# aswanthabam/JPEG_Decoder

Hardware: AMD Instinct MI355X
Metric: Mpixels/s decoded (IDCT+colour) (higher is better)
Workload: dtype f32; 1 GPU; stream of 4096x4096 baseline 4:4:4 images, 32 images per step (one launch) per GPU, coefficient blocks resident in HBM; sampling=4:4:4, parallelism=images sharded x1, no collective, launched_by=bench.py

## Files before the change

jpeg_decoder_amd/csrc/jb_api.cpp:

```cpp
#include <atomic>
#include <condition_variable>
#include <deque>
#include <map>
#include <memory>
#include <mutex>
#include <thread>
#include <hip/hip_runtime_api.h>

#include <cstdarg>
#include <chrono>
#include <cstdio>
#include <cstdlib>
#include <cstring>
#include <new>
#include <string>
#include <vector>

#include <sched.h>

#include "../../include/jpegblk.h"
#include "jb_kernels.h"
#include "jb_huff.h"
#include "jb_knobs.h"

// ... 715 lines not shown
    size_t cap = lay.device_total + lay.device_total / 4 + 65536;
    if (cap < ctx->blob_hint) cap = ctx->blob_hint;
    JB_HIP(ctx, hipMalloc(&s.d_blob, cap));
    s.blob_cap = cap;
    ctx->blob_hint = cap;
  }
  if (!s.h_status) {
    JB_HIP(ctx, hipHostMalloc((void **)&s.h_status, 4 * 256, hipHostMallocDefault));
    JB_HIP(ctx, hipMalloc((void **)&s.d_status, 4 * 256));
  }
  if (lay.total <= ((size_t)4 << 20)) JB_HIP(ctx, jbk_huff_fetch(s.d_blob, h, lay.total, up));
  else JB_HIP(ctx, hipMemcpyAsync(s.d_blob, h, lay.total, hipMemcpyHostToDevice, up));
  JB_HIP(ctx, jbk_huff_zero(d_out, zero_bytes, up, s.d_status, 4 * (size_t)lay.n));
  JbHuffLaunch p;
  memset(&p, 0, sizeof p);
  const uint8_t *d = (const uint8_t *)s.d_blob;
  uint8_t *dw = (uint8_t *)s.d_blob;
  p.scan = d + lay.off_scan;
  p.starts = (const uint32_t *)(d + lay.off_starts);
  p.tables = (const JbHuffTables *)(d + lay.off_tab);
  p.images = (const JbHuffImage *)(d + lay.off_img);
  p.wgs = (const JbHuffWg *)(d + lay.off_wg);
  p.sync_wgs = (const JbHuffWg *)(d + lay.off_sync_wg);
  p.coef = d_out;
  p.status = s.d_status;
  p.n_wgs = (int32_t)lay.n_wg;
  p.n_sync_wgs = (int32_t)lay.n_sync_wg;
  p.chunks = (const JbChunkDesc *)(d + lay.off_chunks);
  p.entry = (JbChunkState *)(dw + lay.off_entry);
  p.exit = (JbChunkState *)(dw + lay.off_exit);
  p.cps = (uint32_t *)(dw + lay.off_cps);
  p.chunk_dc = (JbChunkDc *)(dw + lay.off_chunk_dc);
  p.wgsum = (JbWgSum *)(dw + lay.off_wgsum);
  p.n_chunks_total = lay.n_chunks;
  p.sync_launches = lay.n_sync_wg > 0 && lay.n_wg == lay.n ? 1 : sync_launches;
  p.max_chunk_bytes = lay.max_chunk_bytes;
  p.max_tabs = lay.max_tabs;
  JB_HIP(ctx, jbk_huff_launch(p, up));
  return JB_OK;
}

int pack_into_slot(jb_ctx *ctx, Slot &s, const JbHuffJob *const *jobs, int n, int64_t coef_stride, JbHuffLayout *lay) {
  const size_t need = jb_huff_pack_size_(jobs, n);
  if (need > s.h_blob_cap) {
    if (s.h_blob) (void)hipHostFree(s.h_blob);
    s.h_blob = nullptr, s.h_blob_cap = 0;
    const size_t cap = need + need / 4 + 65536;
    JB_HIP(ctx, hipHostMalloc((void **)&s.h_blob, cap, hipHostMallocDefault));
    s.h_blob_cap = cap;
  }
  const int rc = jb_huff_pack_(jobs, n, coef_stride, s.h_blob, lay);
  return rc ? fail(ctx, rc, "submission too large for the device entropy decoder") : JB_OK;
}

int submit_jobs_impl(jb_ctx *ctx, const JbHuffJob *const *jobs, const uint8_t *packed, const JbHuffLayout *lay_in,
                     const jb_image_desc *desc_in, const uint16_t *qtabs_in, int n_images, uint8_t *rgb, int64_t rgb_stride,
                     uint32_t *status_out, int *ticket, bool dst_device = false, int scale = 1, const jb_output_spec *fmt = nullptr) {
  if (ctx->n_slots == 0) return fail(ctx, JB_ERR_CAPACITY, "context was created without staging buffers");
  if (n_images < 1 || n_images > kMaxBatch) return fail(ctx, JB_ERR_GEOMETRY, "n_images = %d outside 1..%d", n_images, kMaxBatch);
  const jb_image_desc *desc = jobs ? &jobs[0]->desc : desc_in;
  jb_geometry g;
  int rc = check_desc(ctx, desc, &g);
  if (rc) return rc;
  int32_t out_w = 0, out_h = 0;
  if (jb_scaled_size(desc->width, desc->height, scale, &out_w, &out_h) != JB_OK) return fail(ctx, JB_ERR_GEOMETRY, "scale %d is not 1, 2, 4 or 8", scale);
  const int64_t out_bytes = 3LL * out_w * out_h * fmt_esize(fmt);
// ... 392 lines not shown
      Entry fresh;
      CPU_ZERO(&fresh.set);
      fresh.n = numa_cpus_for_(device, numa_knob, &fresh.set);
      it = cache.emplace(std::make_pair(device, numa_knob), fresh).first;
    }
    e = it->second;
  }
  if (e.n <= 0) return 0;
  if (sched_setaffinity(0, sizeof e.set, &e.set) != 0) return 0;
  return e.n;
}

void jb_ctx_set_last_desc_(jb_ctx *ctx, const jb_image_desc *d) { ctx->last_desc = *d; }
const JbKnobs *jb_ctx_knobs_(const jb_ctx *ctx) { return &ctx->knobs; }

int jb_fail_(jb_ctx *ctx, int code, const char *msg) { return fail(ctx, code, "%s", msg); }

size_t jb_huff_pack_size_(const JbHuffJob *const *jobs, int n) {
  size_t n_wg = 0, n_starts = 0, scan_bytes = 0, n_chunks = 0;
  for (int i = 0; i < n; i++) {
    n_wg += (jobs[i]->img.n_chunks + kJbOwnChunks - 1) / kJbOwnChunks;
    n_chunks += jobs[i]->img.n_chunks;
    n_starts += jobs[i]->starts.size();
    scan_bytes += ((jobs[i]->scan.size() + 15) & ~(size_t)15);
  }
  return (size_t)n * sizeof(JbHuffImage) + 2 * n_wg * sizeof(JbHuffWg) + (size_t)n * sizeof(JbHuffTables) + n_starts * 4 +
         n_chunks * sizeof(JbChunkDesc) + scan_bytes + 512;
}

int jb_huff_pack_(const JbHuffJob *const *jobs, int n, int64_t coef_stride, uint8_t *h, JbHuffLayout *lay) {
  auto a16 = [](size_t v) { return (v + 15) & ~(size_t)15; };
  std::vector<int> set_of((size_t)n, 0);
  std::vector<int> sets;
  size_t n_wg = 0, n_sync_wg = 0, n_starts = 0, scan_bytes = 0, n_chunks = 0;
  lay->max_chunk_bytes = 0;
  lay->max_tabs = 0;
  for (int i = 0; i < n; i++) {
    int found = -1;
    for (size_t k = 0; k < sets.size() && found < 0; k++)
      if (jobs[sets[k]]->n_tabs == jobs[i]->n_tabs && memcmp(&jobs[sets[k]]->tables, &jobs[i]->tables, sizeof(JbHuffTables)) == 0) found = (int)k;
    if (found < 0) {
      found = (int)sets.size();
      sets.push_back(i);
    }
    set_of[(size_t)i] = found;
    const size_t wgs = (jobs[i]->img.n_chunks + kJbOwnChunks - 1) / kJbOwnChunks;
    n_wg += wgs;
    if (jobs[i]->img.needs_sync) n_sync_wg += wgs;
    n_chunks += jobs[i]->img.n_chunks;
    n_starts += jobs[i]->starts.size();
    scan_bytes += a16(jobs[i]->scan.size());
    if (jobs[i]->img.chunk_bytes > lay->max_chunk_bytes) lay->max_chunk_bytes = jobs[i]->img.chunk_bytes;
    if (jobs[i]->n_tabs > lay->max_tabs) lay->max_tabs = jobs[i]->n_tabs;
    if ((int64_t)jobs[i]->geo.coef_bytes > coef_stride) return JB_ERR_CAPACITY;
  }
  lay->off_img = 0;
  lay->off_wg = a16((size_t)n * sizeof(JbHuffImage));
  lay->off_sync_wg = a16(lay->off_wg + n_wg * sizeof(JbHuffWg));
  lay->off_tab = a16(lay->off_sync_wg + n_sync_wg * sizeof(JbHuffWg));
  lay->off_starts = lay->off_tab + sets.size() * sizeof(JbHuffTables);
  lay->off_chunks = a16(lay->off_starts + n_starts * 4);
  lay->off_scan = a16(lay->off_chunks + n_chunks * sizeof(JbChunkDesc));
  lay->total = lay->off_scan + scan_bytes + 256;
  lay->off_entry = a16(lay->total);
  lay->off_exit = a16(lay->off_entry + n_chunks * sizeof(JbChunkState));
  lay->off_cps = a16(lay->off_exit + n_chunks * sizeof(JbChunkState));
  lay->off_chunk_dc = (a16(lay->off_cps + n_chunks * kJbCheckpoints * 4) + 31) & ~(size_t)31;
  lay->off_wgsum = lay->off_chunk_dc + n_chunks * sizeof(JbChunkDc);
  lay->device_total = a16(lay->off_wgsum + n_wg * sizeof(JbWgSum));
  lay->n = n;
  lay->n_wg = (int)n_wg;
  lay->n_sync_wg = (int)n_sync_wg;
  lay->n_chunks = (uint32_t)n_chunks;
  lay->coef_stride = coef_stride;
  if (lay->device_total > 0xffffff00u || n_wg > 0x7fffffffu || n_chunks > 0x3fffffffu) return JB_ERR_CAPACITY;
  JbHuffImage *im = (JbHuffImage *)(h + lay->off_img);
  JbHuffWg *wg = (JbHuffWg *)(h + lay->off_wg);
  JbHuffWg *swg = (JbHuffWg *)(h + lay->off_sync_wg);
  uint32_t *st = (uint32_t *)(h + lay->off_starts);
  size_t w = 0, sw = 0, si = 0, sc = lay->off_scan, chunk0 = 0;
  for (size_t k = 0; k < sets.size(); k++) memcpy(h + lay->off_tab + k * sizeof(JbHuffTables), &jobs[sets[k]]->tables, sizeof(JbHuffTables));
  for (int i = 0; i < n; i++) {
    const JbHuffJob &j = *jobs[i];
    im[i] = j.img;
    im[i].scan_off = (uint32_t)(sc - lay->off_scan);
    im[i].int_off = (uint32_t)si;
    im[i].table_set = (uint32_t)set_of[(size_t)i];
    im[i].coef_off = (int64_t)i * coef_stride;
    im[i].state_off = (uint32_t)chunk0;
    im[i].wg0 = (uint32_t)w;
    JbChunkDesc *cd = (JbChunkDesc *)(h + lay->off_chunks) + chunk0;
    uint32_t c = 0;
    for (uint32_t seg = 0; seg + 1 < (uint32_t)j.starts.size(); seg++) {
      const uint32_t k = jb_chunks_of_(j.starts[seg + 1] - j.starts[seg], j.img.chunk_bytes);
      if (c + k > j.img.n_chunks) return JB_ERR_STATE;
      for (uint32_t q = 0; q < k; q++) cd[c++] = JbChunkDesc{j.starts[seg] + q * j.img.chunk_bytes, seg | (q == 0 ? 0x80000000u : 0u)};
    }
    if (c != j.img.n_chunks) return JB_ERR_STATE;
    chunk0 += j.img.n_chunks;
    for (uint32_t f = 0; f < j.img.n_chunks; f += kJbOwnChunks) {
      wg[w++] = JbHuffWg{(uint32_t)i, f};
      if (j.img.needs_sync) swg[sw++] = JbHuffWg{(uint32_t)i, f};
    }
    memcpy(st + si, j.starts.data(), j.starts.size() * 4);
    si += j.starts.size();
    memcpy(h + sc, j.scan.data(), j.scan.size());
    sc += a16(j.scan.size());
  }
  memset(h + sc, 0, 256);
  return JB_OK;
}
```

jpeg_decoder_amd/csrc/jb_frontend.cpp:

```cpp
#include <chrono>
#include <cstdio>
#include <cstdlib>
#include <cstring>
#include <memory>
#include <string>
#include <thread>
#include <vector>

#include "../../include/jpegblk.h"
#include "jb_entropy.h"
#include "jb_hostmem.h"
#include "jb_huff.h"
#include "jb_huff_core.h"
#include "jb_knobs.h"

struct jb_ctx;
int jb_fail_(jb_ctx *ctx, int code, const char *msg);
void jb_ctx_set_last_desc_(jb_ctx *ctx, const jb_image_desc *d);
const JbKnobs *jb_ctx_knobs_(const jb_ctx *ctx);
extern "C" int jb_decode_job_(jb_ctx *ctx, const JbHuffJob *job, uint8_t *rgb, int64_t rgb_stride);
extern "C" int jb_decode_job_scaled_(jb_ctx *ctx, const JbHuffJob *job, uint8_t *rgb, int64_t rgb_stride, int scale);
extern "C" int jb_blocks_to_rgb_scaled_(jb_ctx *ctx, const jb_image_desc *desc, const int16_t *coef, const uint16_t *qtabs,
                                        uint8_t *rgb, int64_t rgb_stride, int scale);
extern "C" int jb_decode_job_fmt_(jb_ctx *ctx, const JbHuffJob *job, uint8_t *rgb, int64_t rgb_stride, int scale, const jb_output_spec *fmt);
// ... 279 lines not shown
      const HuffTable &t = is_ac ? fr->ac[ac_ids[q]] : fr->dc[dc_ids[q - n_ac]];
      if (!jb_huff_fill_table_(t.counts, t.symbols, is_ac, &job->tables, (uint32_t)q, job->n_tabs, &n_t2))
        return done(JB_ERR_UNSUPPORTED, "Huffman tables with more long codes than the device decoder's tables hold: host decoder");
    }
  }
  const uint32_t ny = (uint32_t)(fr->desc.hs * fr->desc.vs);
  job->img.nb = fr->ncomp == 1 ? 1u : ny + 2;
  job->img.lut_ac = job->img.lut_dc = job->img.lut_comp = 0;
  for (uint32_t b = 0; b < job->img.nb; b++) {
    const uint32_t c = b < ny ? 0u : b - ny + 1u;
    job->img.lut_ac |= (uint32_t)ac_slot[c] << (4 * b);
    job->img.lut_dc |= (uint32_t)(n_ac + dc_slot[c]) << (4 * b);
    job->img.lut_comp |= c << (4 * b);
  }
  static thread_local CleanScan tls_scan;
  CleanScan &cs = tls_scan;
  unstuff(fr->scan, fr->scan + fr->scan_len, cs);
  if ((int64_t)cs.n_intervals() != n_int) return done(JB_ERR_UNSUPPORTED, "restart markers do not match the frame: host decoder");
  if (cs.start.back() > 0x0ffff000u) return done(JB_ERR_UNSUPPORTED, "scan too large for 32-bit bit offsets: host decoder");
  job->scan_len = cs.start.back();
  job->scan.assign(cs.bytes.begin(), cs.bytes.begin() + (long)(job->scan_len + 64));
  job->starts.resize(cs.start.size());
  for (size_t i = 0; i < cs.start.size(); i++) job->starts[i] = (uint32_t)cs.start[i];
  job->img.scan_off = job->img.int_off = job->img.table_set = 0;
  job->img.scan_len = (uint32_t)job->scan_len;
  job->img.n_int = (uint32_t)n_int;
  job->img.ri = (uint32_t)(ri > 0 ? ri : n_mcus);
  job->img.n_mcus = (uint32_t)n_mcus;
  job->img.coef_off = 0;
  job->img.blk_bytes = fr->ncomp == 1 ? 384u : 128u;
  job->img.wg0 = 0;
  if ((uint64_t)n_mcus * job->img.nb >= (1u << 24)) return done(JB_ERR_UNSUPPORTED, "more blocks than the device decoder's 24-bit block index holds: host decoder");
  job->img.n_blocks = (uint32_t)(n_mcus * job->img.nb);
  const uint32_t chunk_bytes = (chunk_knob == 64 || chunk_knob == 128) ? chunk_knob : kJbChunkBytes;
  job->img.chunk_bytes = chunk_bytes;
  {
    uint64_t n_chunks = 0;
    bool needs_sync = false;
    for (size_t i = 0; i + 1 < job->starts.size(); i++) {
      if (job->starts[i + 1] < job->starts[i]) return done(JB_ERR_FORMAT, "restart intervals out of order");
      const uint32_t k = jb_chunks_of_(job->starts[i + 1] - job->starts[i], chunk_bytes);
      needs_sync |= k > 1;
      n_chunks += k;
    }
    if (n_chunks > 0x3fffffffu) return done(JB_ERR_UNSUPPORTED, "scan too large for the device decoder: host decoder");
    job->img.n_chunks = (uint32_t)n_chunks;
    job->img.needs_sync = needs_sync ? 1u : 0u;
  }
  job->img.state_off = 0;
  if (ri == 0 && job->scan_len == 0) return done(JB_ERR_FORMAT, "empty scan");
  return done(JB_OK, "");
}

extern "C" {

int jb_entropy_decode(const uint8_t *jpeg, size_t jpeg_bytes, jb_image_desc *desc, uint16_t *qtabs,
                      int16_t *coef, size_t coef_cap_bytes) {
  return jb_entropy_decode_mt(jpeg, jpeg_bytes, desc, qtabs, coef, coef_cap_bytes, 1);
}

int jb_entropy_decode_mt(const uint8_t *jpeg, size_t jpeg_bytes, jb_image_desc *desc, uint16_t *qtabs,
                         int16_t *coef, size_t coef_cap_bytes, int n_threads) {
  if (!jpeg || !desc) return jb_fail_(nullptr, JB_ERR_NULL, "jb_entropy_decode: NULL pointer");
  Frame *fr = new Frame();
  Err e;
  int rc = parse_headers(jpeg, jpeg_bytes, *fr, e);
// ... 161 lines not shown
```

jpeg_decoder_amd/csrc/jb_huff.h:

```cpp
#pragma once
#include <stdint.h>

constexpr int kJbT1Bits = 10;
constexpr int kJbT2Bits = 16 - kJbT1Bits;
constexpr uint32_t kJbT1Entries = 1u << kJbT1Bits;
constexpr uint32_t kJbT2Entries = 1u << kJbT2Bits;
constexpr uint32_t kJbT2Tables = 24;
constexpr uint32_t kJbMaxTabs = 6;
struct JbHuffTables {
  uint16_t t1[kJbMaxTabs][kJbT1Entries];
  uint16_t t2[kJbT2Tables][kJbT2Entries];
};
constexpr uint32_t kJbAdvEob = 82;

struct JbHuffImage {
  uint32_t scan_off;
  uint32_t scan_len;
  uint32_t int_off;
  uint32_t n_int;
  uint32_t ri;
  uint32_t n_mcus;
  uint32_t nb;
  uint32_t table_set;
  int64_t coef_off;
  uint32_t lut_ac;
  uint32_t lut_dc;
  uint32_t lut_comp;
  uint32_t n_chunks;
  uint32_t state_off;
  uint32_t n_blocks;
  uint32_t chunk_bytes;
  uint32_t wg0;
  uint32_t needs_sync;
  uint32_t blk_bytes;
  uint32_t n_tabs;
};

struct JbHuffWg {
  uint32_t image;
  uint32_t first_chunk;
};

constexpr uint32_t kJbChunkBytes = 128;
constexpr int kJbHuffLanes = 256;
constexpr uint32_t kJbWarmChunks = 8;
constexpr uint32_t kJbOwnChunks = kJbHuffLanes - kJbWarmChunks;
constexpr int kJbSyncLaunches = 2;
constexpr int kJbSyncLaunchesMax = 8;

inline uint32_t jb_chunks_of_(uint32_t interval_bytes, uint32_t chunk_bytes) { return interval_bytes ? (interval_bytes + chunk_bytes - 1) / chunk_bytes : 1u; }
struct JbChunkDesc {
  uint32_t start;
  uint32_t seg;
};

struct JbChunkState {
  uint32_t bitpos;
  uint32_t meta;
};

constexpr uint32_t kJbCheckpointBits = 256;
constexpr uint32_t kJbCheckpoints = 4;

struct JbWgSum {
  uint32_t has_first;
  uint32_t blocks;
  uint32_t dc[3];
  uint32_t pad[3];
};
struct JbChunkDc {
  uint32_t dc[3];
  uint32_t first_block;
  uint32_t count;
  uint32_t pad[3];
};

struct JbHuffLaunch {
  const uint8_t *scan;
  const uint32_t *starts;
  const JbHuffTables *tables;
  const JbHuffImage *images;
  const JbHuffWg *wgs;
  const JbHuffWg *sync_wgs;
  int16_t *coef;
  uint32_t *status;
  int32_t n_wgs;
  int32_t n_sync_wgs;
  const JbChunkDesc *chunks;
  JbChunkState *entry;
  JbChunkState *exit;
  uint32_t *cps;
  JbChunkDc *chunk_dc;
  JbWgSum *wgsum;
  uint32_t n_chunks_total;
  int32_t sync_launches;
  uint32_t max_chunk_bytes;
  uint32_t max_tabs;
};


#include <string>
#include <vector>

#include "../../include/jpegblk.h"

struct JbHuffJob {
  jb_image_desc desc;
  jb_geometry geo;
  uint16_t qtabs[256];
  JbHuffImage img;
  JbHuffTables tables;
  uint32_t n_tabs = 0;
  std::vector<uint8_t> scan;
  size_t scan_len = 0;
  std::vector<uint32_t> starts;
};
int jb_huff_prepare_(const uint8_t *jpeg, size_t jpeg_bytes, JbHuffJob *job, std::string *err, uint32_t chunk_bytes = 0);

struct JbHuffLayout {
  size_t off_img = 0, off_wg = 0, off_sync_wg = 0, off_tab = 0, off_starts = 0, off_chunks = 0, off_scan = 0, total = 0;
  size_t off_entry = 0, off_exit = 0, off_cps = 0, off_chunk_dc = 0, off_wgsum = 0, device_total = 0;
  int n = 0, n_wg = 0, n_sync_wg = 0;
  uint32_t n_chunks = 0, max_chunk_bytes = 0, max_tabs = 0;
  int64_t coef_stride = 0;
};
inline bool jb_huff_worth_it_(const JbHuffJob &job, uint32_t min_chunks) { return job.img.n_chunks >= min_chunks; }
size_t jb_huff_pack_size_(const JbHuffJob *const *jobs, int n);
int jb_huff_pack_(const JbHuffJob *const *jobs, int n, int64_t coef_stride, uint8_t *dst, JbHuffLayout *lay);
bool jb_huff_fill_table_(const uint8_t counts[17], const uint8_t *symbols, bool is_ac, JbHuffTables *set, uint32_t tix, uint32_t n_tabs, uint32_t *n_t2);
```

jpeg_decoder_amd/csrc/jb_huff.hip:

```cpp
#include <hip/hip_runtime.h>
#include <stdint.h>

#include "jb_huff_core.h"
#include "jb_kernels.h"

namespace {

constexpr uint32_t L = kJbhLanes;
constexpr int kMaxPasses = (int)L + 4;

__constant__ uint8_t kZz2Dev[64] = {0,   2,   16,  32,  18,  4,   6,   20,  34,  48, 64,  50,  36,  22,  8,   10,
                                    24,  38,  52,  66,  80,  96,  82,  68,  54,  40, 26,  12,  14,  28,  42,  56,
                                    70,  84,  98,  112, 114, 100, 86,  72,  58,  44, 30,  46,  60,  74,  88,  102,
                                    116, 118, 104, 90,  76,  62,  78,  92,  106, 120, 122, 108, 94,  110, 124, 126};

template <uint32_t kMaxChunk>
struct Lay {
  static constexpr uint32_t kRows = jbh_rows(kMaxChunk);
  static constexpr uint32_t kNcp = kMaxChunk * 8u / kJbCheckpointBits;
  static_assert(kNcp <= kJbCheckpoints, "records per chunk");
  static constexpr uint32_t off_stream = 0;
  static constexpr uint32_t off_cp = off_stream + kRows * L * 4u;
  static constexpr uint32_t off_xbit = off_cp + kNcp * L * 4u;
  static constexpr uint32_t off_xmeta = off_xbit + L * 4u;
// ... 148 lines not shown
  const bool owned = tid >= kJbWarmChunks && ci < img.n_chunks;
  const bool active = ci < img.n_chunks && (owned || launch == 0);
  const uint32_t gidx = img.state_off + (ci < img.n_chunks ? ci : img.n_chunks - 1u);
  const ChunkGeo g = chunk_geo(p, img, gidx);
  const uint32_t u0 = jbh_u_of_bit(g.start, g.start * 8u), u_end = u0 + (g.end - g.start) * 8u;
  const size_t n_all = p.n_chunks_total;

  JbChunkState entry{g.start * 8u, 0u}, exitst{0u, 0u};
  bool changed = active;
  if (launch > 0) {
    bool c0 = false;
    JbChunkState ne{0u, 0u};
    if (tid == kJbWarmChunks && owned && !g.first) {
      ne = p.exit[gidx - 1u];
      const JbChunkState en = p.entry[gidx];
      c0 = ne.bitpos != en.bitpos || ((ne.meta ^ en.meta) & 0xffffu) != 0;
    }
    if (!__syncthreads_or(c0)) return;
    entry = p.entry[gidx];
    exitst = p.exit[gidx];
    changed = c0;
    if (c0) entry = JbChunkState{ne.bitpos, ne.meta & 0xffffu};
  }
  load_tables(tab, p, img, tid);
  if (active) load_stream<Ly::kRows>(stream, p.scan + img.scan_off, g.start, tid);
#pragma unroll
  for (uint32_t i = 0; i < Ly::kNcp; i++) cpst[i * L + tid] = launch > 0 ? p.cps[i * n_all + gidx] : 0xffffffffu;
  __syncthreads();

  JbhCtx cx;
  cx.scol = stream + tid;
  cx.tab = tab;
  cx.zz2 = nullptr;
  cx.lut_ac = img.lut_ac, cx.lut_dc = img.lut_dc, cx.lut_comp = img.lut_comp;
  cx.nb4 = img.nb * 4u;
  cx.blk_bytes = img.blk_bytes;
  cx.t2_first = img.n_tabs * kJbT1Entries;
  uint32_t *const cpl = cpst + tid;

  for (int pass = 0; pass < kMaxPasses; pass++) {
    if (__builtin_amdgcn_ballot_w64(changed) != 0) {
      JbhLane st;
      {
        const uint32_t bit = entry.bitpos < g.start * 8u ? g.start * 8u : entry.bitpos;
        const uint32_t u = jbh_u_of_bit(g.start, bit);
        st.u = (changed && u < u_end) ? u : u_end;
        st.k = entry.meta & 0xffu;
        st.blk4 = ((entry.meta >> 8) & 0xffu) * 4u;
        if (st.k > 63u) st.k = 0;
        if (st.blk4 >= cx.nb4) st.blk4 = 0;
        st.nblk = 0;
      }
      uint32_t none = 0;
      while (st.u < u_end) {
        const uint32_t up = st.u;
        (void)jbh_step<false>(cx, st, none, none, none, nullptr, 0u);
        if (((st.u ^ up) >> 8) != 0) {
          uint32_t *rec = cpl + ((st.u >> 8) - 1u) * L;
          const uint32_t s = jbh_pack_state(st), old = *rec;
          const bool met = (st.u < u_end) & (((old ^ s) & 0xfffffu) == 0);
          *rec = met ? old : s;
          st.u = met ? (kMet | ((st.u >> 8) - 1u)) : st.u;
        }
      }
      JBH_TRACE_PASS_END(pass);
      if (changed) {
        if (st.u >= kMet) {
// ... 58 lines not shown
  const uint32_t bpi = img.ri * img.nb;

  load_tables(tab, p, img, tid);
  if (tid < 16) ((uint32_t *)misc)[tid] = ((const uint32_t *)kZz2Dev)[tid];
  if (active) load_stream<Ly::kRows>(stream, p.scan + img.scan_off, g.start, tid);

  uint32_t err = 0;
  JbChunkState entry{g.start * 8u, 0u}, want{0u, 0u};
  uint32_t block = g.seg * bpi;
  if (img.needs_sync) {
    Seg mine{0, 0, 0, 0, 0};
    if (active) {
      want = p.exit[gidx];
      mine.f = g.first ? 1u : 0u;
      mine.n = (want.meta >> 16) + (g.first ? g.seg * bpi : 0u);
      if (!g.first) {
        const JbChunkState prev = p.exit[gidx - 1u];
        const JbChunkState en = p.entry[gidx];
        entry = JbChunkState{prev.bitpos, prev.meta & 0xffffu};
        if (en.bitpos != prev.bitpos || ((en.meta ^ prev.meta) & 0xffffu) != 0) err |= 4u;
      }
    }
    const Seg carry = fold_left_workgroups(p, img.wg0, img.wg0 + wg.first_chunk / kJbOwnChunks, misc + 40, tid);
    Seg total;
    const Seg left = scan_left(mine, carry, misc + 16, tid, &total);
    if (!g.first) block = left.n;
  }
  __syncthreads();

  JbhCtx cx;
  cx.scol = stream + tid;
  cx.tab = tab;
  cx.zz2 = (const uint8_t *)misc;
  cx.lut_ac = img.lut_ac, cx.lut_dc = img.lut_dc, cx.lut_comp = img.lut_comp;
  cx.nb4 = img.nb * 4u;
  cx.blk_bytes = img.blk_bytes;
  cx.t2_first = img.n_tabs * kJbT1Entries;

  uint32_t block_end = (g.seg + 1u) * img.ri < img.n_mcus ? (g.seg + 1u) * bpi : img.n_mcus * img.nb;
  if (block_end > img.n_blocks) block_end = img.n_blocks;
  JbhLane st;
  const bool overran = active && entry.bitpos > g.end * 8u;
  {
    const uint32_t bit = entry.bitpos < g.start * 8u ? g.start * 8u : entry.bitpos;
    const uint32_t u = jbh_u_of_bit(g.start, bit);
    st.u = u < u_end ? u : u_end;
    st.k = entry.meta & 0xffu;
    st.blk4 = ((entry.meta >> 8) & 0xffu) * 4u;
    if (st.k > 63u) st.k = 0;
    if (st.blk4 >= cx.nb4) st.blk4 = 0;
    st.nblk = 0;
  }
  const uint32_t k_in = st.k;
  uint32_t dc0 = 0, dc1 = 0, dc2 = 0;
  uint8_t *const coef = (uint8_t *)p.coef + img.coef_off;
  bool live = active && st.u < u_end && block < block_end;
  while (live) {
    if (jbh_step<true>(cx, st, dc0, dc1, dc2, coef, block)) {
      err |= 1u;
      live = false;
    } else {
      live = st.u < u_end && block + st.nblk < block_end;
    }
  }
  JBH_TRACE_PASS_END(0);
  if (active) {
    if (g.last) {
      if (block + st.nblk != block_end || st.k != 0 || st.u > u_end || overran) err |= 2u;
    } else if (img.needs_sync) {
      if (jbh_bit_of_u(g.start, st.u) != want.bitpos || (st.k | (st.blk4 << 6) | ((st.nblk & 0xffffu) << 16)) != want.meta) err |= 4u;
    }
    if (err) atomicOr(p.status + wg.image, err);
    JbChunkDc o;
    o.dc[0] = dc0, o.dc[1] = dc1, o.dc[2] = dc2;
    o.first_block = block + (k_in != 0 ? 1u : 0u);
    o.count = err ? 0u : st.nblk + (st.k != 0 ? 1u : 0u) - (k_in != 0 ? 1u : 0u);
    o.pad[0] = o.pad[1] = o.pad[2] = 0;
    p.chunk_dc[gidx] = o;
  }
  if (img.needs_sync) {
    Seg mine{0, 0, 0, 0, 0};
    if (active) mine = Seg{g.first ? 1u : 0u, 0u, dc0, dc1, dc2};
    Seg total;
    (void)seg_scan_wg(mine, misc + 16, tid, &total);
    if (tid == 0) {
      JbWgSum *o = p.wgsum + img.wg0 + wg.first_chunk / kJbOwnChunks;
      o->dc[0] = total.d0, o->dc[1] = total.d1, o->dc[2] = total.d2;
    }
  }
}

__global__ __launch_bounds__(kJbHuffLanes) void jb_huff_dc_kernel(const JbHuffLaunch p) {
  extern __shared__ __attribute__((aligned(16))) uint8_t lds[];
  uint32_t *const misc = (uint32_t *)lds;
  const uint32_t tid = threadIdx.x;
  const JbHuffWg wg = p.wgs[blockIdx.x];
  const JbHuffImage img = p.images[wg.image];
  const uint32_t ci = wg.first_chunk + tid;
  const bool active = tid < kJbOwnChunks && ci < img.n_chunks;
  const uint32_t gidx = img.state_off + (active ? ci : img.n_chunks - 1u);
  const bool first = (p.chunks[gidx].seg >> 31) != 0;
  JbChunkDc cd = p.chunk_dc[gidx];
  if (!active) cd.count = 0;
  uint32_t p0 = 0, p1 = 0, p2 = 0;
  if (img.needs_sync) {
    Seg mine{0, 0, 0, 0, 0};
    if (active) mine = Seg{first ? 1u : 0u, 0u, cd.dc[0], cd.dc[1], cd.dc[2]};
    const Seg carry = fold_left_workgroups(p, img.wg0, img.wg0 + wg.first_chunk / kJbOwnChunks, misc + 40, tid);
    Seg total;
    const Seg left = scan_left(mine, carry, misc + 16, tid, &total);
    if (!first) p0 = left.d0, p1 = left.d1, p2 = left.d2;
  }
  uint8_t *const coef = (uint8_t *)p.coef + img.coef_off;
  uint32_t pos4 = (cd.first_block % img.nb) * 4u;
  uint32_t bad = 0;
  constexpr uint32_t kBatch = 24;
  for (uint32_t i = 0; i < cd.count; i += kBatch) {
    int32_t diff[kBatch];
#pragma unroll
    for (uint32_t q = 0; q < kBatch; q++) diff[q] = i + q < cd.count ? *(const int16_t *)(coef + (size_t)jbh_mul24(cd.first_block + i + q, img.blk_bytes)) : 0;
#pragma unroll
    for (uint32_t q = 0; q < kBatch; q++) {
      if (i + q < cd.count) {
        const uint32_t c = jbh_ubfe(img.lut_comp, pos4, 4);
        const uint32_t pr = (c == 0 ? p0 : c == 1 ? p1 : p2) + (uint32_t)diff[q];
        bad |= (pr + 32768u) > 65535u ? 1u : 0u;
        p0 = c == 0 ? pr : p0;
        p1 = c == 1 ? pr : p1;
        p2 = c == 2 ? pr : p2;
        *(int16_t *)(coef + (size_t)jbh_mul24(cd.first_block + i + q, img.blk_bytes)) = (int16_t)pr;
        pos4 = pos4 + 4u == img.nb * 4u ? 0u : pos4 + 4u;
      }
    }
  }
  if (bad) atomicOr(p.status + wg.image, 1u);
}

__global__ __launch_bounds__(256) void jb_huff_fetch_kernel(uint4 *dst, const uint4 *src, uint32_t n16) {
  for (uint32_t i = blockIdx.x * 256u + threadIdx.x; i < n16; i += gridDim.x * 256u) dst[i] = src[i];
}
__global__ __launch_bounds__(256) void jb_huff_zero_kernel(uint4 *dst, uint64_t n16, uint4 *small, uint32_t small16) {
  const uint4 z = make_uint4(0, 0, 0, 0);
  if (blockIdx.x == 0 && threadIdx.x < small16) small[threadIdx.x] = z;
  for (uint64_t i = (uint64_t)blockIdx.x * 256u + threadIdx.x; i < n16; i += (uint64_t)gridDim.x * 256u) dst[i] = z;
}
hipError_t jbk_huff_zero(void *d_dst, size_t bytes, hipStream_t stream, void *d_small, size_t small_bytes) {
  (void)hipGetLastError();
  const uint64_t n16 = (bytes + 15) / 16;
  uint64_t blocks = (n16 + 255u) / 256u;
  if (blocks > 8192u) blocks = 8192u;
  const uint32_t small16 = d_small ? (uint32_t)((small_bytes + 15) / 16) : 0u;
  if (small16 > 256u) return hipErrorInvalidValue;
  hipLaunchKernelGGL(jb_huff_zero_kernel, dim3((unsigned)(blocks ? blocks : 1u)), dim3(256), 0, stream, (uint4 *)d_dst, n16, (uint4 *)d_small, small16);
  return hipGetLastError();
}
hipError_t jbk_huff_fetch(void *d_dst, const void *h_pinned_src, size_t bytes, hipStream_t stream) {
  (void)hipGetLastError();
  const uint32_t n16 = (uint32_t)((bytes + 15) / 16);
  unsigned blocks = (n16 + 255u) / 256u;
  if (blocks > 1024u) blocks = 1024u;
  hipLaunchKernelGGL(jb_huff_fetch_kernel, dim3(blocks ? blocks : 1u), dim3(256), 0, stream, (uint4 *)d_dst, (const uint4 *)h_pinned_src, n16);
  return hipGetLastError();
}

// ... 21 lines not shown
```

jpeg_decoder_amd/csrc/jb_huff_core.h:

```cpp
#pragma once
#include <stdint.h>

#include "jb_huff.h"

#if defined(__HIPCC__)
#define JBH_FN __host__ __device__ inline __attribute__((always_inline))
#else
#define JBH_FN inline
#endif

JBH_FN uint32_t jbh_alignbit(uint32_t hi, uint32_t lo, uint32_t sh) {
#if defined(__HIP_DEVICE_COMPILE__)
  return __builtin_amdgcn_alignbit(hi, lo, sh);
#else
  return (uint32_t)(((((uint64_t)hi) << 32) | lo) >> (sh & 31u));
#endif
}
JBH_FN uint32_t jbh_ubfe(uint32_t v, uint32_t off, uint32_t width) {
#if defined(__HIP_DEVICE_COMPILE__)
  return __builtin_amdgcn_ubfe(v, off, width);
#else
  off &= 31u, width &= 31u;
  return width ? (v >> off) & ((1u << width) - 1u) : 0u;
#endif
}
JBH_FN int32_t jbh_sbfe(uint32_t v, uint32_t off, uint32_t width) {
#if defined(__HIP_DEVICE_COMPILE__)
  return __builtin_amdgcn_sbfe((int32_t)v, off, width);
#else
  off &= 31u, width &= 31u;
  if (!width) return 0;
  const uint32_t f = (v >> off) & ((1u << width) - 1u);
  return (int32_t)(f << (32u - width)) >> (32u - width);
#endif
}

JBH_FN uint32_t jbh_mul24(uint32_t a, uint32_t b) { return (a & 0xffffffu) * (b & 0xffffffu); }

#ifndef JBH_TRACE_STEP
#define JBH_TRACE_STEP() ((void)0)
#define JBH_TRACE_PASS_END(pass) ((void)0)
#endif

constexpr uint32_t kJbhLanes = (uint32_t)kJbHuffLanes;
constexpr uint32_t jbh_rows(uint32_t chunk_bytes) { return chunk_bytes / 4u + 3u; }

JBH_FN uint32_t jbh_base_byte(uint32_t start) { return (start & ~3u) - 4u; }
JBH_FN uint32_t jbh_u_of_bit(uint32_t start, uint32_t bit) { return bit - 8u * jbh_base_byte(start) - 1u; }
JBH_FN uint32_t jbh_bit_of_u(uint32_t start, uint32_t u) { return u + 8u * jbh_base_byte(start) + 1u; }

struct JbhCtx {
  const uint32_t *scol;
  const uint16_t *tab;
  const uint8_t *zz2;
  uint32_t lut_ac, lut_dc, lut_comp;
  uint32_t nb4;
  uint32_t blk_bytes;
  uint32_t t2_first;
};
struct JbhLane {
  uint32_t u;
  uint32_t k;
  uint32_t blk4;
  uint32_t nblk;
};

template <bool kStore>
JBH_FN bool jbh_step(const JbhCtx &cx, JbhLane &st, uint32_t &dc0, uint32_t &dc1, uint32_t &dc2, uint8_t *coef, uint32_t block0) {
  JBH_TRACE_STEP();
  const uint32_t u = st.u;
  const uint32_t j = jbh_ubfe(u, 5, 27);
  const uint32_t w = jbh_alignbit(cx.scol[j * kJbhLanes], cx.scol[j * kJbhLanes + kJbhLanes], ~u);
  const bool isdc = st.k == 0;
  const uint32_t tix = jbh_ubfe(isdc ? cx.lut_dc : cx.lut_ac, st.blk4, 4);
  uint32_t e = cx.tab[(tix << kJbT1Bits) + (w >> (32 - kJbT1Bits))];
  if (e - 1u < 31u)
    e = cx.tab[cx.t2_first + ((e - 1u) << kJbT2Bits) + ((w >> 16) & (kJbT2Entries - 1u))];
  const uint32_t total = e & 31u, size = (e >> 5) & 15u, adv = e >> 9;
  const uint32_t k1 = st.k + adv;
  const bool bad = e == 0 || (k1 - 65u) < 17u;
  if (kStore) {
    const int32_t x = jbh_sbfe(w, 32u - total, size);
    const int32_t val = x - (int32_t)(((1u << size) - 1u) ^ (uint32_t)(x >> 31));
    const uint32_t c = jbh_ubfe(cx.lut_comp, st.blk4, 4);
    const uint32_t dcv = (isdc && !bad) ? (uint32_t)val : 0u;
    dc0 += c == 0 ? dcv : 0u;
    dc1 += c == 1 ? dcv : 0u;
    dc2 += c == 2 ? dcv : 0u;
    if (!bad && (isdc || size != 0))
      *(int16_t *)(coef + (jbh_mul24(block0 + st.nblk, cx.blk_bytes) + cx.zz2[k1 - 1u])) = (int16_t)val;
  }
  const uint32_t k2 = k1 - ((size == 0 && !isdc) ? 1u : 0u);
  const bool done = k2 >= 64u;
  const bool next = done || bad;
  st.k = next ? 0u : k2;
  st.nblk += (done && !bad) ? 1u : 0u;
  const uint32_t b4 = st.blk4 + (next ? 4u : 0u);
  st.blk4 = b4 == cx.nb4 ? 0u : b4;
  st.u = u + (bad ? 1u : total);
  return bad;
}

JBH_FN uint32_t jbh_pack_state(const JbhLane &st) { return st.u | (st.k << 11) | (st.blk4 << 15) | (st.nblk << 20); }

#include <string.h>

inline uint16_t jbh_entry_(bool is_ac, int len, int sym) {
  if (!is_ac) {
    if (sym > 11) return 0;
    return (uint16_t)((len + sym) | (sym << 5) | (1 << 9));
  }
  const int run = sym >> 4, size = sym & 15;
  if (size > 10) return 0;
  if (sym == 0) return (uint16_t)(len | (kJbAdvEob << 9));
  if (sym == 0xf0) return (uint16_t)(len | (17 << 9));
  return (uint16_t)((len + size) | (size << 5) | ((run + 1) << 9));
}

inline bool jb_huff_fill_table_impl_(const uint8_t counts[17], const uint8_t *symbols, bool is_ac, JbHuffTables *set, uint32_t tix, uint32_t n_tabs,
                                     uint32_t *n_t2) {
  uint16_t *t1 = set->t1[tix];
  memset(t1, 0, sizeof set->t1[0]);
  uint32_t code = 0;
// ... 29 lines not shown
```

Before: 645,900 Mpixels/s.

## Stage DC differences in a compact side array for the DC prefix kernel

Measured after the change: 645,400 Mpixels/s (median of 2 runs). No clear change (-0.1%).

```diff
diff --git a/jpeg_decoder_amd/csrc/jb_api.cpp b/jpeg_decoder_amd/csrc/jb_api.cpp
--- a/jpeg_decoder_amd/csrc/jb_api.cpp
+++ b/jpeg_decoder_amd/csrc/jb_api.cpp
@@ -771,6 +771,8 @@
   p.cps = (uint32_t *)(dw + lay.off_cps);
   p.chunk_dc = (JbChunkDc *)(dw + lay.off_chunk_dc);
   p.wgsum = (JbWgSum *)(dw + lay.off_wgsum);
+  p.dc = (int16_t *)(dw + lay.off_dc);
+  p.dc_to_blocks = 1;
   p.n_chunks_total = lay.n_chunks;
   p.sync_launches = lay.n_sync_wg > 0 && lay.n_wg == lay.n ? 1 : sync_launches;
   p.max_chunk_bytes = lay.max_chunk_bytes;
@@ -1229,7 +1231,7 @@
   auto a16 = [](size_t v) { return (v + 15) & ~(size_t)15; };
   std::vector<int> set_of((size_t)n, 0);
   std::vector<int> sets;
-  size_t n_wg = 0, n_sync_wg = 0, n_starts = 0, scan_bytes = 0, n_chunks = 0;
+  size_t n_wg = 0, n_sync_wg = 0, n_starts = 0, scan_bytes = 0, n_chunks = 0, n_dc = 0;
   lay->max_chunk_bytes = 0;
   lay->max_tabs = 0;
   for (int i = 0; i < n; i++) {
@@ -1245,6 +1247,7 @@
     n_wg += wgs;
     if (jobs[i]->img.needs_sync) n_sync_wg += wgs;
     n_chunks += jobs[i]->img.n_chunks;
+    n_dc += ((size_t)jobs[i]->img.n_blocks + 7) & ~(size_t)7;
     n_starts += jobs[i]->starts.size();
     scan_bytes += a16(jobs[i]->scan.size());
     if (jobs[i]->img.chunk_bytes > lay->max_chunk_bytes) lay->max_chunk_bytes = jobs[i]->img.chunk_bytes;
@@ -1264,18 +1267,19 @@
   lay->off_cps = a16(lay->off_exit + n_chunks * sizeof(JbChunkState));
   lay->off_chunk_dc = (a16(lay->off_cps + n_chunks * kJbCheckpoints * 4) + 31) & ~(size_t)31;
   lay->off_wgsum = lay->off_chunk_dc + n_chunks * sizeof(JbChunkDc);
-  lay->device_total = a16(lay->off_wgsum + n_wg * sizeof(JbWgSum));
+  lay->off_dc = a16(lay->off_wgsum + n_wg * sizeof(JbWgSum));
+  lay->device_total = a16(lay->off_dc + n_dc * 2 + 64);
   lay->n = n;
   lay->n_wg = (int)n_wg;
   lay->n_sync_wg = (int)n_sync_wg;
   lay->n_chunks = (uint32_t)n_chunks;
   lay->coef_stride = coef_stride;
-  if (lay->device_total > 0xffffff00u || n_wg > 0x7fffffffu || n_chunks > 0x3fffffffu) return JB_ERR_CAPACITY;
+  if (lay->device_total > 0xffffff00u || n_wg > 0x7fffffffu || n_chunks > 0x3fffffffu || n_dc > 0xffffff00u) return JB_ERR_CAPACITY;
   JbHuffImage *im = (JbHuffImage *)(h + lay->off_img);
   JbHuffWg *wg = (JbHuffWg *)(h + lay->off_wg);
   JbHuffWg *swg = (JbHuffWg *)(h + lay->off_sync_wg);
   uint32_t *st = (uint32_t *)(h + lay->off_starts);
-  size_t w = 0, sw = 0, si = 0, sc = lay->off_scan, chunk0 = 0;
+  size_t w = 0, sw = 0, si = 0, sc = lay->off_scan, chunk0 = 0, dc0 = 0;
   for (size_t k = 0; k < sets.size(); k++) memcpy(h + lay->off_tab + k * sizeof(JbHuffTables), &jobs[sets[k]]->tables, sizeof(JbHuffTables));
   for (int i = 0; i < n; i++) {
     const JbHuffJob &j = *jobs[i];
@@ -1286,6 +1290,8 @@
     im[i].coef_off = (int64_t)i * coef_stride;
     im[i].state_off = (uint32_t)chunk0;
     im[i].wg0 = (uint32_t)w;
+    im[i].dc_off = (uint32_t)dc0;
+    dc0 += ((size_t)j.img.n_blocks + 7) & ~(size_t)7;
     JbChunkDesc *cd = (JbChunkDesc *)(h + lay->off_chunks) + chunk0;
     uint32_t c = 0;
     for (uint32_t seg = 0; seg + 1 < (uint32_t)j.starts.size(); seg++) {
diff --git a/jpeg_decoder_amd/csrc/jb_frontend.cpp b/jpeg_decoder_amd/csrc/jb_frontend.cpp
--- a/jpeg_decoder_amd/csrc/jb_frontend.cpp
+++ b/jpeg_decoder_amd/csrc/jb_frontend.cpp
@@ -335,6 +335,8 @@
   job->img.wg0 = 0;
   if ((uint64_t)n_mcus * job->img.nb >= (1u << 24)) return done(JB_ERR_UNSUPPORTED, "more blocks than the device decoder's 24-bit block index holds: host decoder");
   job->img.n_blocks = (uint32_t)(n_mcus * job->img.nb);
+  if ((uint64_t)job->img.n_blocks * job->img.blk_bytes >= ((uint64_t)1 << 32))
+    return done(JB_ERR_UNSUPPORTED, "more bytes of blocks than the device decoder's 32-bit block offset holds: host decoder");
   const uint32_t chunk_bytes = (chunk_knob == 64 || chunk_knob == 128) ? chunk_knob : kJbChunkBytes;
   job->img.chunk_bytes = chunk_bytes;
   {
diff --git a/jpeg_decoder_amd/csrc/jb_huff.h b/jpeg_decoder_amd/csrc/jb_huff.h
--- a/jpeg_decoder_amd/csrc/jb_huff.h
+++ b/jpeg_decoder_amd/csrc/jb_huff.h
@@ -34,6 +34,7 @@
   uint32_t needs_sync;
   uint32_t blk_bytes;
   uint32_t n_tabs;
+  uint32_t dc_off;
 };
 
 struct JbHuffWg {
@@ -96,6 +97,8 @@
   int32_t sync_launches;
   uint32_t max_chunk_bytes;
   uint32_t max_tabs;
+  int16_t *dc;
+  uint32_t dc_to_blocks;
 };
 
 
@@ -119,7 +122,7 @@
 
 struct JbHuffLayout {
   size_t off_img = 0, off_wg = 0, off_sync_wg = 0, off_tab = 0, off_starts = 0, off_chunks = 0, off_scan = 0, total = 0;
-  size_t off_entry = 0, off_exit = 0, off_cps = 0, off_chunk_dc = 0, off_wgsum = 0, device_total = 0;
+  size_t off_entry = 0, off_exit = 0, off_cps = 0, off_chunk_dc = 0, off_wgsum = 0, off_dc = 0, device_total = 0;
   int n = 0, n_wg = 0, n_sync_wg = 0;
   uint32_t n_chunks = 0, max_chunk_bytes = 0, max_tabs = 0;
   int64_t coef_stride = 0;
diff --git a/jpeg_decoder_amd/csrc/jb_huff.hip b/jpeg_decoder_amd/csrc/jb_huff.hip
--- a/jpeg_decoder_amd/csrc/jb_huff.hip
+++ b/jpeg_decoder_amd/csrc/jb_huff.hip
@@ -204,6 +204,7 @@
   cx.scol = stream + tid;
   cx.tab = tab;
   cx.zz2 = nullptr;
+  cx.dc = nullptr;
   cx.lut_ac = img.lut_ac, cx.lut_dc = img.lut_dc, cx.lut_comp = img.lut_comp;
   cx.nb4 = img.nb * 4u;
   cx.blk_bytes = img.blk_bytes;
@@ -329,6 +330,7 @@
   cx.scol = stream + tid;
   cx.tab = tab;
   cx.zz2 = (const uint8_t *)misc;
+  cx.dc = p.dc + img.dc_off;
   cx.lut_ac = img.lut_ac, cx.lut_dc = img.lut_dc, cx.lut_comp = img.lut_comp;
   cx.nb4 = img.nb * 4u;
   cx.blk_bytes = img.blk_bytes;
@@ -387,6 +389,7 @@
   }
 }
 
+constexpr uint32_t kJbDcBatch = 30;
 __global__ __launch_bounds__(kJbHuffLanes) void jb_huff_dc_kernel(const JbHuffLaunch p) {
   extern __shared__ __attribute__((aligned(16))) uint8_t lds[];
   uint32_t *const misc = (uint32_t *)lds;
@@ -409,24 +412,37 @@
     if (!first) p0 = left.d0, p1 = left.d1, p2 = left.d2;
   }
   uint8_t *const coef = (uint8_t *)p.coef + img.coef_off;
+  int16_t *const dc = p.dc + img.dc_off;
+  const bool to_blocks = p.dc_to_blocks != 0;
   uint32_t pos4 = (cd.first_block % img.nb) * 4u;
   uint32_t bad = 0;
-  constexpr uint32_t kBatch = 24;
-  for (uint32_t i = 0; i < cd.count; i += kBatch) {
-    int32_t diff[kBatch];
-#pragma unroll
-    for (uint32_t q = 0; q < kBatch; q++) diff[q] = i + q < cd.count ? *(const int16_t *)(coef + (size_t)jbh_mul24(cd.first_block + i + q, img.blk_bytes)) : 0;
-#pragma unroll
-    for (uint32_t q = 0; q < kBatch; q++) {
-      if (i + q < cd.count) {
-        const uint32_t c = jbh_ubfe(img.lut_comp, pos4, 4);
-        const uint32_t pr = (c == 0 ? p0 : c == 1 ? p1 : p2) + (uint32_t)diff[q];
-        bad |= (pr + 32768u) > 65535u ? 1u : 0u;
-        p0 = c == 0 ? pr : p0;
-        p1 = c == 1 ? pr : p1;
-        p2 = c == 2 ? pr : p2;
-        *(int16_t *)(coef + (size_t)jbh_mul24(cd.first_block + i + q, img.blk_bytes)) = (int16_t)pr;
-        pos4 = pos4 + 4u == img.nb * 4u ? 0u : pos4 + 4u;
+  for (uint32_t i = 0; i < cd.count; i += kJbDcBatch) {
+    const uint32_t e0 = cd.first_block + i, mis = e0 & 1u;
+    const uint8_t *src = (const uint8_t *)__builtin_assume_aligned(dc + (e0 - mis), 4);
+    uint32_t d[kJbDcBatch / 2u + 1u];
+#pragma unroll
+    for (uint32_t j = 0; j < 4; j++) {
+      uint4 v;
+      __builtin_memcpy(&v, src + 16u * j, 16);
+      d[4u * j] = v.x, d[4u * j + 1u] = v.y, d[4u * j + 2u] = v.z, d[4u * j + 3u] = v.w;
+    }
+#pragma unroll
+    for (uint32_t q = 0; q < kJbDcBatch; q += 2) {
+      const uint32_t w = jbh_alignbit(d[q / 2u + 1u], d[q / 2u], mis * 16u);
+#pragma unroll
+      for (uint32_t h = 0; h < 2; h++) {
+        if (i + q + h < cd.count) {
+          const uint32_t diff = (uint32_t)jbh_sbfe(w, 16u * h, 16);
+          const uint32_t c = jbh_ubfe(img.lut_comp, pos4, 4);
+          const uint32_t pr = (c == 0 ? p0 : c == 1 ? p1 : p2) + diff;
+          bad |= (pr + 32768u) > 65535u ? 1u : 0u;
+          p0 = c == 0 ? pr : p0;
+          p1 = c == 1 ? pr : p1;
+          p2 = c == 2 ? pr : p2;
+          if (to_blocks) *(int16_t *)(coef + (size_t)jbh_mul24(e0 + q + h, img.blk_bytes)) = (int16_t)pr;
+          else dc[e0 + q + h] = (int16_t)pr;
+          pos4 = pos4 + 4u == img.nb * 4u ? 0u : pos4 + 4u;
+        }
       }
     }
   }
diff --git a/jpeg_decoder_amd/csrc/jb_huff_core.h b/jpeg_decoder_amd/csrc/jb_huff_core.h
--- a/jpeg_decoder_amd/csrc/jb_huff_core.h
+++ b/jpeg_decoder_amd/csrc/jb_huff_core.h
@@ -57,6 +57,7 @@
   uint32_t nb4;
   uint32_t blk_bytes;
   uint32_t t2_first;
+  int16_t *dc;
 };
 struct JbhLane {
   uint32_t u;
@@ -87,8 +88,11 @@
     dc0 += c == 0 ? dcv : 0u;
     dc1 += c == 1 ? dcv : 0u;
     dc2 += c == 2 ? dcv : 0u;
-    if (!bad && (isdc || size != 0))
-      *(int16_t *)(coef + (jbh_mul24(block0 + st.nblk, cx.blk_bytes) + cx.zz2[k1 - 1u])) = (int16_t)val;
+    if (!bad) {
+      if (isdc) cx.dc[block0 + st.nblk] = (int16_t)val;
+      else if (size != 0)
+        *(int16_t *)(coef + (jbh_mul24(block0 + st.nblk, cx.blk_bytes) + cx.zz2[k1 - 1u])) = (int16_t)val;
+    }
   }
   const uint32_t k2 = k1 - ((size == 0 && !isdc) ? 1u : 0u);
   const bool done = k2 >= 64u;
```

## Store DC diffs in a compact side buffer and accumulate per-component sums arithmetically

Applied to the files above, without the earlier changes.

Result: no change. 656,500 Mpixels/s before, 652,000 Mpixels/s after (-0.7%).

```diff
diff --git a/jpeg_decoder_amd/csrc/jb_api.cpp b/jpeg_decoder_amd/csrc/jb_api.cpp
--- a/jpeg_decoder_amd/csrc/jb_api.cpp
+++ b/jpeg_decoder_amd/csrc/jb_api.cpp
@@ -771,6 +771,7 @@
   p.cps = (uint32_t *)(dw + lay.off_cps);
   p.chunk_dc = (JbChunkDc *)(dw + lay.off_chunk_dc);
   p.wgsum = (JbWgSum *)(dw + lay.off_wgsum);
+  p.dc_diff = (int16_t *)(dw + lay.off_dc_diff);
   p.n_chunks_total = lay.n_chunks;
   p.sync_launches = lay.n_sync_wg > 0 && lay.n_wg == lay.n ? 1 : sync_launches;
   p.max_chunk_bytes = lay.max_chunk_bytes;
@@ -1230,6 +1231,7 @@
   std::vector<int> set_of((size_t)n, 0);
   std::vector<int> sets;
   size_t n_wg = 0, n_sync_wg = 0, n_starts = 0, scan_bytes = 0, n_chunks = 0;
+  size_t n_dc = 0;
   lay->max_chunk_bytes = 0;
   lay->max_tabs = 0;
   for (int i = 0; i < n; i++) {
@@ -1245,6 +1247,7 @@
     n_wg += wgs;
     if (jobs[i]->img.needs_sync) n_sync_wg += wgs;
     n_chunks += jobs[i]->img.n_chunks;
+    n_dc += ((size_t)jobs[i]->img.n_blocks + 7) & ~(size_t)7;
     n_starts += jobs[i]->starts.size();
     scan_bytes += a16(jobs[i]->scan.size());
     if (jobs[i]->img.chunk_bytes > lay->max_chunk_bytes) lay->max_chunk_bytes = jobs[i]->img.chunk_bytes;
@@ -1264,7 +1267,8 @@
   lay->off_cps = a16(lay->off_exit + n_chunks * sizeof(JbChunkState));
   lay->off_chunk_dc = (a16(lay->off_cps + n_chunks * kJbCheckpoints * 4) + 31) & ~(size_t)31;
   lay->off_wgsum = lay->off_chunk_dc + n_chunks * sizeof(JbChunkDc);
-  lay->device_total = a16(lay->off_wgsum + n_wg * sizeof(JbWgSum));
+  lay->off_dc_diff = a16(lay->off_wgsum + n_wg * sizeof(JbWgSum));
+  lay->device_total = a16(lay->off_dc_diff + n_dc * sizeof(int16_t) + kJbDcDiffPad);
   lay->n = n;
   lay->n_wg = (int)n_wg;
   lay->n_sync_wg = (int)n_sync_wg;
@@ -1275,7 +1279,7 @@
   JbHuffWg *wg = (JbHuffWg *)(h + lay->off_wg);
   JbHuffWg *swg = (JbHuffWg *)(h + lay->off_sync_wg);
   uint32_t *st = (uint32_t *)(h + lay->off_starts);
-  size_t w = 0, sw = 0, si = 0, sc = lay->off_scan, chunk0 = 0;
+  size_t w = 0, sw = 0, si = 0, sc = lay->off_scan, chunk0 = 0, dc0 = 0;
   for (size_t k = 0; k < sets.size(); k++) memcpy(h + lay->off_tab + k * sizeof(JbHuffTables), &jobs[sets[k]]->tables, sizeof(JbHuffTables));
   for (int i = 0; i < n; i++) {
     const JbHuffJob &j = *jobs[i];
@@ -1285,6 +1289,8 @@
     im[i].table_set = (uint32_t)set_of[(size_t)i];
     im[i].coef_off = (int64_t)i * coef_stride;
     im[i].state_off = (uint32_t)chunk0;
+    im[i].dc_off = (uint32_t)dc0;
+    dc0 += ((size_t)j.img.n_blocks + 7) & ~(size_t)7;
     im[i].wg0 = (uint32_t)w;
     JbChunkDesc *cd = (JbChunkDesc *)(h + lay->off_chunks) + chunk0;
     uint32_t c = 0;
diff --git a/jpeg_decoder_amd/csrc/jb_huff.h b/jpeg_decoder_amd/csrc/jb_huff.h
--- a/jpeg_decoder_amd/csrc/jb_huff.h
+++ b/jpeg_decoder_amd/csrc/jb_huff.h
@@ -34,6 +34,7 @@
   uint32_t needs_sync;
   uint32_t blk_bytes;
   uint32_t n_tabs;
+  uint32_t dc_off;
 };
 
 struct JbHuffWg {
@@ -75,6 +76,7 @@
   uint32_t pad[3];
 };
 
+constexpr uint32_t kJbDcDiffPad = 64;
 struct JbHuffLaunch {
   const uint8_t *scan;
   const uint32_t *starts;
@@ -91,6 +93,7 @@
   JbChunkState *exit;
   uint32_t *cps;
   JbChunkDc *chunk_dc;
+  int16_t *dc_diff;
   JbWgSum *wgsum;
   uint32_t n_chunks_total;
   int32_t sync_launches;
@@ -119,7 +122,7 @@
 
 struct JbHuffLayout {
   size_t off_img = 0, off_wg = 0, off_sync_wg = 0, off_tab = 0, off_starts = 0, off_chunks = 0, off_scan = 0, total = 0;
-  size_t off_entry = 0, off_exit = 0, off_cps = 0, off_chunk_dc = 0, off_wgsum = 0, device_total = 0;
+  size_t off_entry = 0, off_exit = 0, off_cps = 0, off_chunk_dc = 0, off_wgsum = 0, off_dc_diff = 0, device_total = 0;
   int n = 0, n_wg = 0, n_sync_wg = 0;
   uint32_t n_chunks = 0, max_chunk_bytes = 0, max_tabs = 0;
   int64_t coef_stride = 0;
diff --git a/jpeg_decoder_amd/csrc/jb_huff.hip b/jpeg_decoder_amd/csrc/jb_huff.hip
--- a/jpeg_decoder_amd/csrc/jb_huff.hip
+++ b/jpeg_decoder_amd/csrc/jb_huff.hip
@@ -205,6 +205,7 @@
   cx.tab = tab;
   cx.zz2 = nullptr;
   cx.lut_ac = img.lut_ac, cx.lut_dc = img.lut_dc, cx.lut_comp = img.lut_comp;
+  cx.lut_comp2 = 0;
   cx.nb4 = img.nb * 4u;
   cx.blk_bytes = img.blk_bytes;
   cx.t2_first = img.n_tabs * kJbT1Entries;
@@ -330,6 +331,7 @@
   cx.tab = tab;
   cx.zz2 = (const uint8_t *)misc;
   cx.lut_ac = img.lut_ac, cx.lut_dc = img.lut_dc, cx.lut_comp = img.lut_comp;
+  cx.lut_comp2 = jbh_comp_squares(img.lut_comp);
   cx.nb4 = img.nb * 4u;
   cx.blk_bytes = img.blk_bytes;
   cx.t2_first = img.n_tabs * kJbT1Entries;
@@ -351,9 +353,10 @@
   const uint32_t k_in = st.k;
   uint32_t dc0 = 0, dc1 = 0, dc2 = 0;
   uint8_t *const coef = (uint8_t *)p.coef + img.coef_off;
+  int16_t *const dcd = p.dc_diff + img.dc_off;
   bool live = active && st.u < u_end && block < block_end;
   while (live) {
-    if (jbh_step<true>(cx, st, dc0, dc1, dc2, coef, block)) {
+    if (jbh_step<true>(cx, st, dc0, dc1, dc2, coef, block, dcd)) {
       err |= 1u;
       live = false;
     } else {
@@ -361,6 +364,7 @@
     }
   }
   JBH_TRACE_PASS_END(0);
+  jbh_solve_dc_sums(dc0, dc1, dc2);
   if (active) {
     if (g.last) {
       if (block + st.nblk != block_end || st.k != 0 || st.u > u_end || overran) err |= 2u;
@@ -409,18 +413,20 @@
     if (!first) p0 = left.d0, p1 = left.d1, p2 = left.d2;
   }
   uint8_t *const coef = (uint8_t *)p.coef + img.coef_off;
+  const int16_t *const dcd = p.dc_diff + img.dc_off;
   uint32_t pos4 = (cd.first_block % img.nb) * 4u;
   uint32_t bad = 0;
   constexpr uint32_t kBatch = 24;
+  static_assert(kBatch * 2u <= kJbDcDiffPad, "the pad behind dc_diff");
   for (uint32_t i = 0; i < cd.count; i += kBatch) {
-    int32_t diff[kBatch];
-#pragma unroll
-    for (uint32_t q = 0; q < kBatch; q++) diff[q] = i + q < cd.count ? *(const int16_t *)(coef + (size_t)jbh_mul24(cd.first_block + i + q, img.blk_bytes)) : 0;
+    uint32_t d[kBatch / 2u];
+    __builtin_memcpy(d, dcd + (cd.first_block + i), sizeof d);
 #pragma unroll
     for (uint32_t q = 0; q < kBatch; q++) {
       if (i + q < cd.count) {
+        const uint32_t diff = (uint32_t)jbh_sbfe(d[q >> 1], (q & 1u) * 16u, 16);
         const uint32_t c = jbh_ubfe(img.lut_comp, pos4, 4);
-        const uint32_t pr = (c == 0 ? p0 : c == 1 ? p1 : p2) + (uint32_t)diff[q];
+        const uint32_t pr = (c == 0 ? p0 : c == 1 ? p1 : p2) + diff;
         bad |= (pr + 32768u) > 65535u ? 1u : 0u;
         p0 = c == 0 ? pr : p0;
         p1 = c == 1 ? pr : p1;
diff --git a/jpeg_decoder_amd/csrc/jb_huff_core.h b/jpeg_decoder_amd/csrc/jb_huff_core.h
--- a/jpeg_decoder_amd/csrc/jb_huff_core.h
+++ b/jpeg_decoder_amd/csrc/jb_huff_core.h
@@ -36,6 +36,7 @@
 }
 
 JBH_FN uint32_t jbh_mul24(uint32_t a, uint32_t b) { return (a & 0xffffffu) * (b & 0xffffffu); }
+JBH_FN int32_t jbh_mul24s(int32_t a, int32_t b) { return jbh_sbfe((uint32_t)a, 0, 24) * jbh_sbfe((uint32_t)b, 0, 24); }
 
 #ifndef JBH_TRACE_STEP
 #define JBH_TRACE_STEP() ((void)0)
@@ -54,6 +55,7 @@
   const uint16_t *tab;
   const uint8_t *zz2;
   uint32_t lut_ac, lut_dc, lut_comp;
+  uint32_t lut_comp2;
   uint32_t nb4;
   uint32_t blk_bytes;
   uint32_t t2_first;
@@ -64,9 +66,14 @@
   uint32_t blk4;
   uint32_t nblk;
 };
+JBH_FN uint32_t jbh_comp_squares(uint32_t lut_comp) { return (lut_comp & 0x11111111u) | ((lut_comp & 0x22222222u) << 1); }
+JBH_FN void jbh_solve_dc_sums(uint32_t &dc0, uint32_t &dc1, uint32_t &dc2) {
+  const uint32_t s2 = (uint32_t)((int32_t)(dc2 - dc1) >> 1), s1 = dc1 - 2u * s2, s0 = dc0 - s1 - s2;
+  dc0 = s0, dc1 = s1, dc2 = s2;
+}
 
 template <bool kStore>
-JBH_FN bool jbh_step(const JbhCtx &cx, JbhLane &st, uint32_t &dc0, uint32_t &dc1, uint32_t &dc2, uint8_t *coef, uint32_t block0) {
+JBH_FN bool jbh_step(const JbhCtx &cx, JbhLane &st, uint32_t &dc0, uint32_t &dc1, uint32_t &dc2, uint8_t *coef, uint32_t block0, int16_t *dcd = nullptr) {
   JBH_TRACE_STEP();
   const uint32_t u = st.u;
   const uint32_t j = jbh_ubfe(u, 5, 27);
@@ -82,13 +89,17 @@
   if (kStore) {
     const int32_t x = jbh_sbfe(w, 32u - total, size);
     const int32_t val = x - (int32_t)(((1u << size) - 1u) ^ (uint32_t)(x >> 31));
-    const uint32_t c = jbh_ubfe(cx.lut_comp, st.blk4, 4);
-    const uint32_t dcv = (isdc && !bad) ? (uint32_t)val : 0u;
-    dc0 += c == 0 ? dcv : 0u;
-    dc1 += c == 1 ? dcv : 0u;
-    dc2 += c == 2 ? dcv : 0u;
-    if (!bad && (isdc || size != 0))
-      *(int16_t *)(coef + (jbh_mul24(block0 + st.nblk, cx.blk_bytes) + cx.zz2[k1 - 1u])) = (int16_t)val;
+    if (!bad) {
+      const uint32_t blk = block0 + st.nblk;
+      if (isdc) {
+        dcd[blk] = (int16_t)val;
+        dc0 += (uint32_t)val;
+        dc1 += (uint32_t)jbh_mul24s(val, (int32_t)jbh_ubfe(cx.lut_comp, st.blk4, 4));
+        dc2 += (uint32_t)jbh_mul24s(val, (int32_t)jbh_ubfe(cx.lut_comp2, st.blk4, 4));
+      } else if (size != 0) {
+        *(int16_t *)(coef + (jbh_mul24(blk, cx.blk_bytes) + cx.zz2[k1 - 1u])) = (int16_t)val;
+      }
+    }
   }
   const uint32_t k2 = k1 - ((size == 0 && !isdc) ? 1u : 0u);
   const bool done = k2 >= 64u;
```
